# mbzuai-oryx/Video-LLaVA

Measured on NVIDIA H100. Metric: videos/sec (100-frame CLIP encode + 7B 32-tok decode), higher is better.
Workload: dtype bf16

## Files before the change

### video-llava_b200/csrc/attention_tc.cu

```cuda
#include "common.cuh"
#include "kernels.h"

#include <stdlib.h>

namespace vcl {

namespace {

constexpr int VA_WG = 2;
constexpr int VA_THREADS = VA_WG * 128;
constexpr int VA_TILE = 64 * 128;
constexpr int VA_KEY_TILES = 5;
constexpr int VA_OFF_K = 0;
constexpr int VA_OFF_VT = VA_OFF_K + VA_KEY_TILES * VA_TILE;
constexpr int VA_OFF_Q = VA_OFF_VT + VA_KEY_TILES * VA_TILE;
constexpr int VA_OFF_P = VA_OFF_Q + VA_WG * VA_TILE;
constexpr int VA_OFF_BAR = VA_OFF_P + VA_WG * VA_KEY_TILES * VA_TILE;
constexpr int VA_SMEM = VA_OFF_BAR + 64 + 1024;
static_assert(VA_SMEM <= 227 * 1024, "shared memory");

__device__ __forceinline__ uint32_t va_sw128(int row, int chunk) {
  return (uint32_t)row * 128u + (uint32_t)((chunk ^ (row & 7)) << 4);
}

__device__ __forceinline__ void named_bar_sync_wg(int id) { asm volatile("bar.sync %0, 128;" ::"r"(id) : "memory"); }

__global__ void __launch_bounds__(VA_THREADS, 1)
attn_vit_tc_kernel(const __grid_constant__ CUtensorMap tmap, const bf16* __restrict__ qkv, bf16* __restrict__ out,
                   int S, int H, int C) {
  extern __shared__ uint8_t smem_raw[];
  const uint32_t raw_addr = smem_u32(smem_raw);
  const uint32_t pad = ((raw_addr + 1023u) & ~1023u) - raw_addr;
  uint8_t* smem = smem_raw + pad;
  const uint32_t sbase = raw_addr + pad;
  const uint32_t kbar = sbase + VA_OFF_BAR;
  auto qbar = [&](int w) { return sbase + VA_OFF_BAR + 8u * (1 + w); };

  const int frame = blockIdx.x / H, h = blockIdx.x - frame * H;
  const int row0 = frame * S;
  const int wg = threadIdx.x >> 7, t = threadIdx.x & 127, lane = threadIdx.x & 31, wq = t >> 5;
  const int n_qt = (S + 63) / 64;
  const int n_kt = (S + 63) / 64;

  if (threadIdx.x == 0) {
    tma_prefetch_desc(&tmap);
    mbar_init(kbar, 1);
    for (int w = 0; w < VA_WG; ++w) mbar_init(qbar(w), 1);
    mbar_fence_init();
  }
  __syncthreads();
  if (threadIdx.x == 0) {
    mbar_arrive_expect_tx(kbar, n_kt * VA_TILE);
    for (int i = 0; i < n_kt; ++i) tma_load_2d(sbase + VA_OFF_K + i * VA_TILE, &tmap, kbar, C + h * 64, row0 + 64 * i);
    for (int w = 0; w < VA_WG && w < n_qt; ++w) {
      mbar_arrive_expect_tx(qbar(w), VA_TILE);
      tma_load_2d(sbase + VA_OFF_Q + w * VA_TILE, &tmap, qbar(w), h * 64, row0 + 64 * w);
    }
  }
  const bf16* vg = qkv + (long long)row0 * 3 * C + 2 * C + h * 64;
  for (int idx = threadIdx.x; idx < VA_KEY_TILES * 64 * 8; idx += VA_THREADS) {
    const int key = idx % (VA_KEY_TILES * 64), c = idx / (VA_KEY_TILES * 64);
    uint4 v = make_uint4(0u, 0u, 0u, 0u);
    if (key < S) v = *reinterpret_cast<const uint4*>(vg + (long long)key * 3 * C + c * 8);
    const uint32_t w4[4] = {v.x, v.y, v.z, v.w};
    uint8_t* tile = smem + VA_OFF_VT + (key >> 6) * VA_TILE;
    const int kc = (key & 63) >> 3, ke = key & 7;
#pragma unroll
    for (int e = 0; e < 8; ++e) {
      const uint16_t hv = (uint16_t)(e & 1 ? w4[e >> 1] >> 16 : w4[e >> 1] & 0xffffu);
      *reinterpret_cast<uint16_t*>(tile + va_sw128(c * 8 + e, kc) + ke * 2) = hv;
    }
  }
  asm volatile("fence.proxy.async.shared::cta;" ::: "memory");
  __syncthreads();
  mbar_wait(kbar, 0);

  const int r0 = 16 * wq + (lane >> 2), c2 = 2 * (lane & 3);
  const bool tail = S > 256;
  uint8_t* P = smem + VA_OFF_P + wg * VA_KEY_TILES * VA_TILE;
  const uint32_t p_addr = sbase + VA_OFF_P + wg * VA_KEY_TILES * VA_TILE;
  const uint32_t q_addr = sbase + VA_OFF_Q + wg * VA_TILE;
  uint32_t qphase = 0;
  float s[128], s2[16], o[32];
  for (int qt = wg; qt < n_qt; qt += VA_WG) {
    mbar_wait(qbar(wg), qphase);
    qphase ^= 1u;
#pragma unroll
    for (int i = 0; i < 128; ++i) s[i] = 0.f;
#pragma unroll
    for (int i = 0; i < 16; ++i) s2[i] = 0.f;
    wgmma_fence();
#pragma unroll
    for (int k = 0; k < 4; ++k) {
      const uint64_t ad = wgmma_desc_k_sw128(q_addr) + 2u * k;
      wgmma_bf16<256>(s, ad, wgmma_desc_k_sw128(sbase + VA_OFF_K) + 2u * k, k > 0 ? 1u : 0u);
      if (tail) wgmma_bf16<32>(s2, ad, wgmma_desc_k_sw128(sbase + VA_OFF_K + 256 * 128) + 2u * k, k > 0 ? 1u : 0u);
    }
    wgmma_commit();
    wgmma_wait<0>();
    wgmma_fence_regs(s);
    wgmma_fence_regs(s2);
    named_bar_sync_wg(1 + wg);
    if (t == 0 && qt + VA_WG < n_qt) {
      mbar_arrive_expect_tx(qbar(wg), VA_TILE);
      tma_load_2d(q_addr, &tmap, qbar(wg), h * 64, row0 + 64 * (qt + VA_WG));
    }
    auto sc = [&](float x, int key) { return key < S ? bf16r(bf16r(x) * 0.125f) : -INFINITY; };
    float m[2] = {-INFINITY, -INFINITY};
    uint32_t sp[64], sp2[8];
    auto pack_sc = [&](const float* a, int i, int key0) {
      const int hh = i & 1, col = key0 + 8 * (i >> 1) + c2;
      const float x0 = sc(a[2 * i], col), x1 = sc(a[2 * i + 1], col + 1);
      m[hh] = fmaxf(m[hh], fmaxf(x0, x1));
      return pack_bf16x2(x0, x1);
    };
    if (tail) {
#pragma unroll
      for (int i = 0; i < 8; ++i) sp2[i] = pack_sc(s2, i, 256);
    }
#pragma unroll
    for (int i = 0; i < 64; ++i) sp[i] = pack_sc(s, i, 0);
    float l[2] = {0.f, 0.f};
#pragma unroll
    for (int r = 0; r < 2; ++r) {
      m[r] = fmaxf(m[r], __shfl_xor_sync(0xffffffffu, m[r], 1));
      m[r] = fmaxf(m[r], __shfl_xor_sync(0xffffffffu, m[r], 2));
    }
    auto put_p = [&](uint32_t x2, int i, int key0) {
      const int hh = i & 1, row = r0 + 8 * hh, col = key0 + 8 * (i >> 1) + c2;
      const float p0 = exp2f((bf16lo(x2) - m[hh]) * 1.4426950408889634f);
      const float p1 = exp2f((bf16hi(x2) - m[hh]) * 1.4426950408889634f);
      l[hh] += p0 + p1;
      *reinterpret_cast<uint32_t*>(P + (col >> 6) * VA_TILE + va_sw128(row, (col & 63) >> 3) + (col & 7) * 2) =
          pack_bf16x2(p0, p1);
    };
#pragma unroll
    for (int i = 0; i < 64; ++i) put_p(sp[i], i, 0);
    if (tail) {
#pragma unroll
      for (int i = 0; i < 8; ++i) put_p(sp2[i], i, 256);
    }
    asm volatile("fence.proxy.async.shared::cta;" ::: "memory");
    named_bar_sync_wg(1 + wg);
#pragma unroll
    for (int i = 0; i < 32; ++i) o[i] = 0.f;
    wgmma_fence();
#pragma unroll
    for (int kk = 0; kk < 16; ++kk)
      wgmma_bf16<64>(o, wgmma_desc_k_sw128(p_addr + (kk >> 2) * VA_TILE) + 2u * (kk & 3),
                     wgmma_desc_k_sw128(sbase + VA_OFF_VT + (kk >> 2) * VA_TILE) + 2u * (kk & 3), kk > 0 ? 1u : 0u);
    if (tail)
      wgmma_bf16<64>(o, wgmma_desc_k_sw128(p_addr + 4 * VA_TILE), wgmma_desc_k_sw128(sbase + VA_OFF_VT + 4 * VA_TILE), 1u);
    wgmma_commit();
    wgmma_wait<0>();
    wgmma_fence_regs(o);
#pragma unroll
    for (int r = 0; r < 2; ++r) {
      l[r] += __shfl_xor_sync(0xffffffffu, l[r], 1);
      l[r] += __shfl_xor_sync(0xffffffffu, l[r], 2);
    }
#pragma unroll
    for (int hh = 0; hh < 2; ++hh) {
      const int q = qt * 64 + r0 + 8 * hh;
      if (q < S) {
        const float inv = 1.0f / l[hh];
        bf16* dst = out + (long long)(row0 + q) * C + h * 64 + c2;
#pragma unroll
        for (int j = 0; j < 8; ++j)
          *reinterpret_cast<uint32_t*>(dst + 8 * j) = pack_bf16x2(o[4 * j + 2 * hh] * inv, o[4 * j + 2 * hh + 1] * inv);
      }
    }
  }
}

}

int init_attention_tc_kernels() {
  VCL_CUDA_OK(cudaFuncSetAttribute(attn_vit_tc_kernel, cudaFuncAttributeMaxDynamicSharedMemorySize, VA_SMEM));
  return 0;
}

bool attention_vit_tc_supported(int S) {
  const bool off = getenv("VCL_VIT_ATTN_FLASH") != nullptr;
  return !off && S >= 129 && S <= 257;
}

int launch_attention_vit_tc(const bf16* qkv, bf16* out, int n_frames, int S, int H, int C, cudaStream_t stream) {
  VCL_REQUIRE(C == H * 64, "attention_vit_tc: head_dim must be 64");
  VCL_REQUIRE(S >= 129 && S <= 257, "attention_vit_tc: S=%d outside 129..257", S);
  VCL_REQUIRE(((uintptr_t)qkv % 16) == 0 && ((uintptr_t)out % 16) == 0, "attention_vit_tc: pointers must be 16-byte aligned");
  CUtensorMap tm;
  if (make_tmap_2d(&tm, qkv, (long long)n_frames * S, 3LL * C, 3LL * C, 64) != 0) return -2;
  attn_vit_tc_kernel<<<n_frames * H, VA_THREADS, VA_SMEM, stream>>>(tm, qkv, out, S, H, C);
  VCL_CUDA_OK(cudaGetLastError());
  count_launches(1);
  return 0;
}

}
```

### video-llava_b200/csrc/common.cuh

```cuda
#pragma once

#include <cuda.h>
#include <cuda_bf16.h>
#include <cuda_fp16.h>
#include <cuda_runtime.h>
#include <stdint.h>

namespace vcl {

typedef __nv_bfloat16 bf16;

void set_last_error(const char* fmt, ...);

#define VCL_CUDA_OK(expr)                                                                      \
  do {                                                                                         \
    cudaError_t _e = (expr);                                                                   \
    if (_e != cudaSuccess) {                                                                   \
      ::vcl::set_last_error("%s:%d: %s -> %s", __FILE__, __LINE__, #expr, cudaGetErrorString(_e)); \
      return -2;                                                                               \
    }                                                                                          \
  } while (0)

#define VCL_REQUIRE(cond, ...)                 \
  do {                                         \
    if (!(cond)) {                             \
      ::vcl::set_last_error(__VA_ARGS__);      \
      return -1;                               \
    }                                          \
  } while (0)

__device__ __forceinline__ float bf16r(float x) { return __bfloat162float(__float2bfloat16_rn(x)); }

__device__ __forceinline__ uint32_t pack_bf16x2(float lo, float hi) {
  __nv_bfloat162 v = __floats2bfloat162_rn(lo, hi);
  return *reinterpret_cast<uint32_t*>(&v);
}
__device__ __forceinline__ float bf16lo(uint32_t v) { return __uint_as_float(v << 16); }
__device__ __forceinline__ float bf16hi(uint32_t v) { return __uint_as_float(v & 0xffff0000u); }

__device__ __forceinline__ uint32_t bf16x2_mul(uint32_t a, uint32_t b) {
  __nv_bfloat162 r = __hmul2(*reinterpret_cast<__nv_bfloat162*>(&a), *reinterpret_cast<__nv_bfloat162*>(&b));
  return *reinterpret_cast<uint32_t*>(&r);
}
__device__ __forceinline__ uint32_t bf16x2_add(uint32_t a, uint32_t b) {
  __nv_bfloat162 r = __hadd2(*reinterpret_cast<__nv_bfloat162*>(&a), *reinterpret_cast<__nv_bfloat162*>(&b));
  return *reinterpret_cast<uint32_t*>(&r);
}

__device__ __forceinline__ float warp_sum(float v) {
#pragma unroll
  for (int o = 16; o > 0; o >>= 1) v += __shfl_xor_sync(0xffffffffu, v, o);
  return v;
}
__device__ __forceinline__ float warp_max(float v) {
#pragma unroll
  for (int o = 16; o > 0; o >>= 1) v = fmaxf(v, __shfl_xor_sync(0xffffffffu, v, o));
  return v;
}

__device__ __forceinline__ uint4 ld_nc_v4(const void* p) {
  uint4 r;
  asm volatile("ld.global.nc.L1::no_allocate.v4.u32 {%0,%1,%2,%3}, [%4];"
               : "=r"(r.x), "=r"(r.y), "=r"(r.z), "=r"(r.w)
               : "l"(p));
  return r;
}

__device__ __forceinline__ uint32_t smem_u32(const void* p) {
  return static_cast<uint32_t>(__cvta_generic_to_shared(p));
}

__device__ __forceinline__ void mbar_init(uint32_t bar, uint32_t count) {
  asm volatile("mbarrier.init.shared::cta.b64 [%0], %1;" ::"r"(bar), "r"(count) : "memory");
}
__device__ __forceinline__ void mbar_fence_init() {
  asm volatile("fence.mbarrier_init.release.cluster;" ::: "memory");
  asm volatile("fence.proxy.async.shared::cta;" ::: "memory");
}
__device__ __forceinline__ void mbar_arrive_expect_tx(uint32_t bar, uint32_t bytes) {
  asm volatile("mbarrier.arrive.expect_tx.shared::cta.b64 _, [%0], %1;" ::"r"(bar), "r"(bytes)
               : "memory");
}
__device__ __forceinline__ void mbar_arrive(uint32_t bar) {
  asm volatile("mbarrier.arrive.shared::cta.b64 _, [%0];" ::"r"(bar) : "memory");
}
__device__ __forceinline__ void mbar_wait(uint32_t bar, uint32_t parity) {
  asm volatile(
      "{\n\t"
      ".reg .pred p;\n\t"
      "VCL_WAIT_%=:\n\t"
      "mbarrier.try_wait.parity.shared::cta.b64 p, [%0], %1;\n\t"
      "@p bra VCL_DONE_%=;\n\t"
      "bra VCL_WAIT_%=;\n\t"
      "VCL_DONE_%=:\n\t"
      "}\n" ::"r"(bar),
      "r"(parity)
      : "memory");
}

__device__ __forceinline__ void tma_prefetch_desc(const void* tmap) {
  asm volatile("prefetch.tensormap [%0];" ::"l"(tmap) : "memory");
}
__device__ __forceinline__ void tma_load_2d(uint32_t dst_smem, const void* tmap, uint32_t bar,
                                            int32_t c0, int32_t c1) {
  asm volatile(
      "cp.async.bulk.tensor.2d.shared::cluster.global.mbarrier::complete_tx::bytes"
      " [%0], [%1, {%3, %4}], [%2];" ::"r"(dst_smem),
      "l"(tmap), "r"(bar), "r"(c0), "r"(c1)
      : "memory");
}

__device__ __forceinline__ void tma_prefetch_2d(const void* tmap, int32_t c0, int32_t c1) {
  asm volatile("cp.async.bulk.prefetch.tensor.2d.L2.global.tile [%0, {%1, %2}];" ::"l"(tmap), "r"(c0), "r"(c1)
               : "memory");
}

__device__ __forceinline__ void tma_load_2d_mc(uint32_t dst_smem, const void* tmap, uint32_t bar,
                                               int32_t c0, int32_t c1, uint16_t cta_mask) {
  asm volatile(
      "cp.async.bulk.tensor.2d.shared::cluster.global.mbarrier::complete_tx::bytes.multicast::cluster"
      " [%0], [%1, {%3, %4}], [%2], %5;" ::"r"(dst_smem),
      "l"(tmap), "r"(bar), "r"(c0), "r"(c1), "h"(cta_mask)
      : "memory");
}

__device__ __forceinline__ uint32_t cluster_ctarank() {
  uint32_t r;
  asm volatile("mov.u32 %0, %%cluster_ctarank;" : "=r"(r));
  return r;
}
__device__ __forceinline__ void cluster_sync_all() {
  asm volatile("barrier.cluster.arrive.release.aligned;" ::: "memory");
  asm volatile("barrier.cluster.wait.acquire.aligned;" ::: "memory");
}

__device__ __forceinline__ uint32_t mapa_cluster(uint32_t smem_addr, uint32_t cta_rank) {
  uint32_t r;
  asm volatile("mapa.shared::cluster.u32 %0, %1, %2;" : "=r"(r) : "r"(smem_addr), "r"(cta_rank));
  return r;
}
__device__ __forceinline__ void mbar_arrive_cluster(uint32_t bar_cluster_addr) {
  asm volatile("mbarrier.arrive.release.cluster.shared::cluster.b64 _, [%0];" ::"r"(bar_cluster_addr) : "memory");
}

__device__ __forceinline__ void wgmma_fence() { asm volatile("wgmma.fence.sync.aligned;" ::: "memory"); }
__device__ __forceinline__ void wgmma_commit() { asm volatile("wgmma.commit_group.sync.aligned;" ::: "memory"); }
template <int N>
__device__ __forceinline__ void wgmma_wait() {
  asm volatile("wgmma.wait_group.sync.aligned %0;" ::"n"(N) : "memory");
}
template <int R>
__device__ __forceinline__ void wgmma_fence_regs(float (&d)[R]) {
#pragma unroll
  for (int i = 0; i < R; ++i) asm volatile("" : "+f"(d[i])::"memory");
}
template <int R>
__device__ __forceinline__ void setmaxnreg_inc() { asm volatile("setmaxnreg.inc.sync.aligned.u32 %0;" ::"n"(R)); }
template <int R>
__device__ __forceinline__ void setmaxnreg_dec() { asm volatile("setmaxnreg.dec.sync.aligned.u32 %0;" ::"n"(R)); }

__device__ __forceinline__ uint64_t wgmma_desc_k_sw128(uint32_t smem_addr) {
  uint64_t d = 0;
  d |= (uint64_t)((smem_addr & 0x3ffffu) >> 4);
  d |= (uint64_t)1 << 16;
  d |= (uint64_t)(1024u >> 4) << 32;
  d |= (uint64_t)1 << 62;
  return d;
}

template <int N>
__device__ __forceinline__ void wgmma_bf16(float (&d)[N / 2], uint64_t adesc, uint64_t bdesc, uint32_t accumulate);
template <>
__device__ __forceinline__ void wgmma_bf16<256>(float (&d)[128], uint64_t adesc, uint64_t bdesc, uint32_t accumulate) {
  asm volatile(
      "{\n\t.reg .pred p;\n\tsetp.ne.b32 p, %130, 0;\n\t"
      "wgmma.mma_async.sync.aligned.m64n256k16.f32.bf16.bf16 {%0, %1, %2, %3, %4, %5, %6, %7, %8, %9, %10, %11, %12, %13, %14, %15, %16, %17, %18, %19, %20, %21, %22, %23, %24, %25, %26, %27, %28, %29, %30, %31, %32, %33, %34, %35, %36, %37, %38, %39, %40, %41, %42, %43, %44, %45, %46, %47, %48, %49, %50, %51, %52, %53, %54, %55, %56, %57, %58, %59, %60, %61, %62, %63, %64, %65, %66, %67, %68, %69, %70, %71, %72, %73, %74, %75, %76, %77, %78, %79, %80, %81, %82, %83, %84, %85, %86, %87, %88, %89, %90, %91, %92, %93, %94, %95, %96, %97, %98, %99, %100, %101, %102, %103, %104, %105, %106, %107, %108, %109, %110, %111, %112, %113, %114, %115, %116, %117, %118, %119, %120, %121, %122, %123, %124, %125, %126, %127}, %128, %129, p, 1, 1, 0, 0;\n\t}"
      : "+f"(d[0]), "+f"(d[1]), "+f"(d[2]), "+f"(d[3]), "+f"(d[4]), "+f"(d[5]), "+f"(d[6]), "+f"(d[7]), "+f"(d[8]), "+f"(d[9]), "+f"(d[10]), "+f"(d[11]), "+f"(d[12]), "+f"(d[13]), "+f"(d[14]), "+f"(d[15]), "+f"(d[16]), "+f"(d[17]), "+f"(d[18]), "+f"(d[19]), "+f"(d[20]), "+f"(d[21]), "+f"(d[22]), "+f"(d[23]), "+f"(d[24]), "+f"(d[25]), "+f"(d[26]), "+f"(d[27]), "+f"(d[28]), "+f"(d[29]), "+f"(d[30]), "+f"(d[31]), "+f"(d[32]), "+f"(d[33]), "+f"(d[34]), "+f"(d[35]), "+f"(d[36]), "+f"(d[37]), "+f"(d[38]), "+f"(d[39]), "+f"(d[40]), "+f"(d[41]), "+f"(d[42]), "+f"(d[43]), "+f"(d[44]), "+f"(d[45]), "+f"(d[46]), "+f"(d[47]), "+f"(d[48]), "+f"(d[49]), "+f"(d[50]), "+f"(d[51]), "+f"(d[52]), "+f"(d[53]), "+f"(d[54]), "+f"(d[55]), "+f"(d[56]), "+f"(d[57]), "+f"(d[58]), "+f"(d[59]), "+f"(d[60]), "+f"(d[61]), "+f"(d[62]), "+f"(d[63]), "+f"(d[64]), "+f"(d[65]), "+f"(d[66]), "+f"(d[67]), "+f"(d[68]), "+f"(d[69]), "+f"(d[70]), "+f"(d[71]), "+f"(d[72]), "+f"(d[73]), "+f"(d[74]), "+f"(d[75]), "+f"(d[76]), "+f"(d[77]), "+f"(d[78]), "+f"(d[79]), "+f"(d[80]), "+f"(d[81]), "+f"(d[82]), "+f"(d[83]), "+f"(d[84]), "+f"(d[85]), "+f"(d[86]), "+f"(d[87]), "+f"(d[88]), "+f"(d[89]), "+f"(d[90]), "+f"(d[91]), "+f"(d[92]), "+f"(d[93]), "+f"(d[94]), "+f"(d[95]), "+f"(d[96]), "+f"(d[97]), "+f"(d[98]), "+f"(d[99]), "+f"(d[100]), "+f"(d[101]), "+f"(d[102]), "+f"(d[103]), "+f"(d[104]), "+f"(d[105]), "+f"(d[106]), "+f"(d[107]), "+f"(d[108]), "+f"(d[109]), "+f"(d[110]), "+f"(d[111]), "+f"(d[112]), "+f"(d[113]), "+f"(d[114]), "+f"(d[115]), "+f"(d[116]), "+f"(d[117]), "+f"(d[118]), "+f"(d[119]), "+f"(d[120]), "+f"(d[121]), "+f"(d[122]), "+f"(d[123]), "+f"(d[124]), "+f"(d[125]), "+f"(d[126]), "+f"(d[127])
      : "l"(adesc), "l"(bdesc), "r"(accumulate));
}
template <>
__device__ __forceinline__ void wgmma_bf16<128>(float (&d)[64], uint64_t adesc, uint64_t bdesc, uint32_t accumulate) {
  asm volatile(
      "{\n\t.reg .pred p;\n\tsetp.ne.b32 p, %66, 0;\n\t"
      "wgmma.mma_async.sync.aligned.m64n128k16.f32.bf16.bf16 {%0, %1, %2, %3, %4, %5, %6, %7, %8, %9, %10, %11, %12, %13, %14, %15, %16, %17, %18, %19, %20, %21, %22, %23, %24, %25, %26, %27, %28, %29, %30, %31, %32, %33, %34, %35, %36, %37, %38, %39, %40, %41, %42, %43, %44, %45, %46, %47, %48, %49, %50, %51, %52, %53, %54, %55, %56, %57, %58, %59, %60, %61, %62, %63}, %64, %65, p, 1, 1, 0, 0;\n\t}"
      : "+f"(d[0]), "+f"(d[1]), "+f"(d[2]), "+f"(d[3]), "+f"(d[4]), "+f"(d[5]), "+f"(d[6]), "+f"(d[7]), "+f"(d[8]), "+f"(d[9]), "+f"(d[10]), "+f"(d[11]), "+f"(d[12]), "+f"(d[13]), "+f"(d[14]), "+f"(d[15]), "+f"(d[16]), "+f"(d[17]), "+f"(d[18]), "+f"(d[19]), "+f"(d[20]), "+f"(d[21]), "+f"(d[22]), "+f"(d[23]), "+f"(d[24]), "+f"(d[25]), "+f"(d[26]), "+f"(d[27]), "+f"(d[28]), "+f"(d[29]), "+f"(d[30]), "+f"(d[31]), "+f"(d[32]), "+f"(d[33]), "+f"(d[34]), "+f"(d[35]), "+f"(d[36]), "+f"(d[37]), "+f"(d[38]), "+f"(d[39]), "+f"(d[40]), "+f"(d[41]), "+f"(d[42]), "+f"(d[43]), "+f"(d[44]), "+f"(d[45]), "+f"(d[46]), "+f"(d[47]), "+f"(d[48]), "+f"(d[49]), "+f"(d[50]), "+f"(d[51]), "+f"(d[52]), "+f"(d[53]), "+f"(d[54]), "+f"(d[55]), "+f"(d[56]), "+f"(d[57]), "+f"(d[58]), "+f"(d[59]), "+f"(d[60]), "+f"(d[61]), "+f"(d[62]), "+f"(d[63])
      : "l"(adesc), "l"(bdesc), "r"(accumulate));
}
template <>
__device__ __forceinline__ void wgmma_bf16<64>(float (&d)[32], uint64_t adesc, uint64_t bdesc, uint32_t accumulate) {
  asm volatile(
      "{\n\t.reg .pred p;\n\tsetp.ne.b32 p, %34, 0;\n\t"
      "wgmma.mma_async.sync.aligned.m64n64k16.f32.bf16.bf16 {%0, %1, %2, %3, %4, %5, %6, %7, %8, %9, %10, %11, %12, %13, %14, %15, %16, %17, %18, %19, %20, %21, %22, %23, %24, %25, %26, %27, %28, %29, %30, %31}, %32, %33, p, 1, 1, 0, 0;\n\t}"
      : "+f"(d[0]), "+f"(d[1]), "+f"(d[2]), "+f"(d[3]), "+f"(d[4]), "+f"(d[5]), "+f"(d[6]), "+f"(d[7]), "+f"(d[8]), "+f"(d[9]), "+f"(d[10]), "+f"(d[11]), "+f"(d[12]), "+f"(d[13]), "+f"(d[14]), "+f"(d[15]), "+f"(d[16]), "+f"(d[17]), "+f"(d[18]), "+f"(d[19]), "+f"(d[20]), "+f"(d[21]), "+f"(d[22]), "+f"(d[23]), "+f"(d[24]), "+f"(d[25]), "+f"(d[26]), "+f"(d[27]), "+f"(d[28]), "+f"(d[29]), "+f"(d[30]), "+f"(d[31])
      : "l"(adesc), "l"(bdesc), "r"(accumulate));
}
template <>
__device__ __forceinline__ void wgmma_bf16<32>(float (&d)[16], uint64_t adesc, uint64_t bdesc, uint32_t accumulate) {
  asm volatile(
      "{\n\t.reg .pred p;\n\tsetp.ne.b32 p, %18, 0;\n\t"
      "wgmma.mma_async.sync.aligned.m64n32k16.f32.bf16.bf16 {%0, %1, %2, %3, %4, %5, %6, %7, %8, %9, %10, %11, %12, %13, %14, %15}, %16, %17, p, 1, 1, 0, 0;\n\t}"
      : "+f"(d[0]), "+f"(d[1]), "+f"(d[2]), "+f"(d[3]), "+f"(d[4]), "+f"(d[5]), "+f"(d[6]), "+f"(d[7]), "+f"(d[8]), "+f"(d[9]), "+f"(d[10]), "+f"(d[11]), "+f"(d[12]), "+f"(d[13]), "+f"(d[14]), "+f"(d[15])
      : "l"(adesc), "l"(bdesc), "r"(accumulate));
}

}
```

### video-llava_b200/csrc/gemm_tc.cu

```cuda
#include "common.cuh"
#include "kernels.h"

#include <cudaTypedefs.h>

namespace vcl {

template <int BLOCK_N>
struct GemmCfg {
  static constexpr int BLOCK_M = 128;
  static constexpr int BLOCK_K = 64;
  static constexpr int A_BYTES = BLOCK_M * BLOCK_K * 2;
  static constexpr int B_BYTES = BLOCK_N * BLOCK_K * 2;
  static constexpr int STAGE_BYTES = A_BYTES + B_BYTES;
  static constexpr int OUT_PITCH = BLOCK_N * 2 + 16;
  static constexpr int OUT_BYTES = BLOCK_M * OUT_PITCH;
  static constexpr int BAR_BYTES = 256;
  static constexpr int STAGES = (BLOCK_N == 256) ? 3 : (BLOCK_N == 128 ? 5 : 8);
  static constexpr int SMEM_BYTES = STAGES * STAGE_BYTES + BAR_BYTES + OUT_BYTES + 1024;
  static_assert((2 * STAGES + 4) * 8 <= BAR_BYTES, "barrier area");
  static_assert(SMEM_BYTES <= 227 * 1024, "shared memory");
};

__device__ __forceinline__ float act_gelu_erf(float x) {
  x = bf16r(x);
// ... 256 lines not shown
          wgmma_bf16<BLOCK_N>(acc, a_desc + 2u * k, b_desc + 2u * k, (kb | k) != 0 ? 1u : 0u);
        }
        wgmma_commit();
        wgmma_wait<1>();
        if (prev >= 0) release(prev);
        prev = stage;
        if (++stage == STAGES) { stage = 0; phase ^= 1u; }
      }
      wgmma_wait<0>();
      release(prev);
      wgmma_fence_regs(acc);
      if (tile != cluster_id) {
        mbar_wait(drained_bar(cw), out_phase);
        out_phase ^= 1u;
      }
      gemm_epilogue_stage<BLOCK_N, ACT>(acc, stg, lane, wq, m_blk * Cfg::BLOCK_M + cw * 64, n_blk, bias, M, N, rope);
      mbar_arrive(staged_bar(cw));
    }
  }

  __syncthreads();
  if (CL > 1) cluster_sync_all();
}

static PFN_cuTensorMapEncodeTiled_v12000 g_encode = nullptr;
static int resolve_encode() {
  if (g_encode) return 0;
  void* fn = nullptr;
  cudaDriverEntryPointQueryResult qres;
  cudaError_t e = cudaGetDriverEntryPoint("cuTensorMapEncodeTiled", &fn, cudaEnableDefault, &qres);
  if (e != cudaSuccess || fn == nullptr || qres != cudaDriverEntryPointSuccess) {
    set_last_error("cuTensorMapEncodeTiled is not available from the driver (%s)",
                   cudaGetErrorString(e));
    return -2;
  }
  g_encode = reinterpret_cast<PFN_cuTensorMapEncodeTiled_v12000>(fn);
  return 0;
}

int make_tmap_2d(CUtensorMap* out, const void* ptr, long long rows, long long cols, long long ld,
                 int box_rows) {
  if (resolve_encode() != 0) return -2;
  cuuint64_t gdim[2] = {(cuuint64_t)cols, (cuuint64_t)rows};
  cuuint64_t gstride[1] = {(cuuint64_t)ld * 2};
  cuuint32_t box[2] = {64u, (cuuint32_t)box_rows};
  cuuint32_t estr[2] = {1u, 1u};
  CUresult r = g_encode(out, CU_TENSOR_MAP_DATA_TYPE_BFLOAT16, 2, const_cast<void*>(ptr), gdim,
                        gstride, box, estr, CU_TENSOR_MAP_INTERLEAVE_NONE,
                        CU_TENSOR_MAP_SWIZZLE_128B, CU_TENSOR_MAP_L2_PROMOTION_L2_256B,
                        CU_TENSOR_MAP_FLOAT_OOB_FILL_NONE);
  if (r != CUDA_SUCCESS) {
    set_last_error("cuTensorMapEncodeTiled failed (%d) ptr=%p rows=%lld cols=%lld ld=%lld box=%d",
                   (int)r, ptr, rows, cols, ld, box_rows);
    return -2;
  }
  return 0;
}

static int g_num_sms = 0;
int device_num_sms() {
  if (g_num_sms == 0) {
    int dev = 0;
    cudaGetDevice(&dev);
    cudaDeviceGetAttribute(&g_num_sms, cudaDevAttrMultiProcessorCount, dev);
    if (g_num_sms <= 0) g_num_sms = 132;
  }
  return g_num_sms;
}

template <int BLOCK_N, int ACT, int CL>
static int launch_one(const GemmArgs& g, cudaStream_t stream) {
  using Cfg = GemmCfg<BLOCK_N>;
  auto kern = gemm_bf16_tn_kernel<BLOCK_N, ACT, CL>;
  CUtensorMap ta, tb;
  if (make_tmap_2d(&ta, g.A, g.M, g.K, g.lda, Cfg::BLOCK_M) != 0) return -2;
  if (make_tmap_2d(&tb, g.W, g.N, g.K, g.ldw, BLOCK_N / CL) != 0) return -2;
  const int num_m = (g.M + 127) / 128;
  const int num_tiles = ((num_m + CL - 1) / CL) * ((g.N + BLOCK_N - 1) / BLOCK_N);
  cudaLaunchConfig_t cfg = {};
  cfg.blockDim = dim3(384);
  cfg.dynamicSmemBytes = Cfg::SMEM_BYTES;
  cfg.stream = stream;
  cudaLaunchAttribute attr[1];
  attr[0].id = cudaLaunchAttributeClusterDimension;
  attr[0].val.clusterDim.x = CL;
  attr[0].val.clusterDim.y = 1;
  attr[0].val.clusterDim.z = 1;
  cfg.attrs = attr;
  cfg.numAttrs = CL > 1 ? 1 : 0;
  static int resident = 0;
  if (resident == 0) {
    if (CL > 1) {
      cfg.gridDim = dim3(CL);
      VCL_CUDA_OK(cudaOccupancyMaxActiveClusters(&resident, kern, &cfg));
    }
    if (resident <= 0) resident = device_num_sms() / CL;
  }
  int clusters = resident;
  if (clusters > num_tiles) clusters = num_tiles;
  if (g.max_ctas > 0 && clusters * CL > g.max_ctas) clusters = g.max_ctas / CL > 0 ? g.max_ctas / CL : 1;
  cfg.gridDim = dim3(clusters * CL);
  VCL_CUDA_OK(cudaLaunchKernelEx(&cfg, kern, ta, tb, g.C, (long long)g.ldc, g.bias, g.residual,
                                 (long long)g.ldr, g.M, g.N, g.K, g.rope));
  count_launches(1);
  return 0;
}
// ... 107 lines not shown
```

### video-llava_b200/csrc/kernels.h

```cpp
#pragma once

#include <cuda.h>
#include <cuda_bf16.h>
#include <cuda_runtime.h>
#include <stdint.h>

namespace vcl {

typedef __nv_bfloat16 bf16;

constexpr int PACK_SEQ_MAX = 64;
constexpr int PACK_HEAD = 6 * PACK_SEQ_MAX;
inline size_t pack_elems(long long rows) { return PACK_HEAD + 2 * (size_t)rows; }
template <class T> __host__ __device__ inline T* pack_off(T* p) { return p; }
template <class T> __host__ __device__ inline T* pack_len(T* p) { return p + PACK_SEQ_MAX; }
template <class T> __host__ __device__ inline T* pack_slot(T* p) { return p + 2 * PACK_SEQ_MAX; }
template <class T> __host__ __device__ inline T* pack_last(T* p) { return p + 3 * PACK_SEQ_MAX; }
template <class T> __host__ __device__ inline T* pack_start(T* p) { return p + 4 * PACK_SEQ_MAX; }
template <class T> __host__ __device__ inline T* pack_end(T* p) { return p + 5 * PACK_SEQ_MAX; }
template <class T> __host__ __device__ inline T* pack_row(T* p, long long r) { return p + PACK_HEAD + 2 * r; }

struct KvPages {
  const int* table = nullptr;
  int row = 0;
  long long blk = 0;
};
__device__ __forceinline__ long long kv_paged_off(const KvPages& p, int slot, int head, int col) {
  return (long long)__ldg(p.table + slot * p.row + (col >> 7)) * p.blk + ((long long)head * 128 + (col & 127)) * 128;
}

enum Act { ACT_NONE = 0, ACT_QGELU = 1, ACT_GELU = 2, ACT_SWIGLU = 3, ACT_ROPE = 4 };
struct RopeEpilogue {
  const bf16* cos_t = nullptr; const bf16* sin_t = nullptr;
  bf16* kcache = nullptr; bf16* vcache = nullptr;
  int S = 0, start_pos = 0, H = 0, s_max = 0;
  const int* n_pad = nullptr;
  const int* pack = nullptr;
  KvPages pages;
};


void set_last_error(const char* fmt, ...);
void count_launches(long long n);
long long launch_count();
int device_num_sms();

struct GemmArgs {
  const bf16* A = nullptr;  long long lda = 0;
  const bf16* W = nullptr;  long long ldw = 0;
  bf16* C = nullptr;        long long ldc = 0;
  const bf16* bias = nullptr;
  const bf16* residual = nullptr; long long ldr = 0;
  int M = 0, N = 0, K = 0;
  int act = ACT_NONE;
  int block_n = 0;
  int cluster = 0;
  int max_ctas = 0;
  RopeEpilogue rope;
};
int launch_gemm_bf16_tn(const GemmArgs& g, cudaStream_t stream);
int init_gemm_kernels();
int make_tmap_2d(CUtensorMap* out, const void* ptr, long long rows, long long cols, long long ld,
                 int box_rows);

int launch_layernorm(const bf16* x, long long ldx, bf16* y, long long ldy, const bf16* w,
                     const bf16* b, int rows, int D, float eps, cudaStream_t stream);
int launch_rmsnorm(const bf16* x, long long ldx, bf16* y, long long ldy, const bf16* w, int rows,
                   int D, float eps, cudaStream_t stream);
int launch_im2col(const void* pixels, int mode, bf16* out, int n_frames, int image, int patch,
                  int KP, cudaStream_t stream);
int launch_clip_embed_ln(const bf16* patch_out, const bf16* cls, const bf16* pos, const bf16* ln_w,
                         const bf16* ln_b, bf16* h, int n_frames, int P, int D, float eps,
                         cudaStream_t stream);
int launch_embed_splice(const long long* ids, const bf16* table, const bf16* vid, const int* vid_start,
                        bf16* h, int B, int S, int D, int n_vid, int vocab, cudaStream_t stream,
                        const int* pack = nullptr, int M = 0);
int launch_rope_table(bf16* cos_t, bf16* sin_t, int max_pos, int head_dim, float theta,
                      cudaStream_t stream);
int launch_rope_kv_prefill(bf16* qkv, bf16* kcache, bf16* vcache, const bf16* cos_t,
                           const bf16* sin_t, int B, int S, int H, int head_dim, int s_max, int pos0,
                           cudaStream_t stream, const int* pos_dev = nullptr, const int* n_pad = nullptr);
int launch_embed_tokens(const int* tok, long long tok_stride, const bf16* table, bf16* h, int B,
                        int D, int vocab, cudaStream_t stream);
int launch_argmax(const float* logits, int* out, long long out_stride, int B, int V,
                  cudaStream_t stream);
int launch_fill_int(int* dst, int value, int n, cudaStream_t stream);

int launch_st_pool(const void* feats, int in_dtype, long long frame_stride, long long patch_stride,
                   int T, int P, int C, int n_temporal, void* out, int out_dtype,
                   cudaStream_t stream);

int launch_cross_entropy(const bf16* logits, long long ld, int V, const long long* labels, long long row0, int rows,
                         int seg, float* nll, bf16* logits_out, cudaStream_t stream);
int launch_nll_mean(const float* nll, const long long* labels, long long rows, int seg, float* nll_out,
                    float* loss_out, cudaStream_t stream);

#ifndef VCL_LOGPROBS_MAX
#define VCL_LOGPROBS_MAX 20
#endif
#ifndef VCL_SAMPLE_WIDE_MAX_V
#define VCL_SAMPLE_WIDE_MAX_V 57344
#endif
struct SampleArgs {
  const float* logits = nullptr; long long ld = 0; int V = 0, B = 0;
  const float* temperature = nullptr; const int* top_k = nullptr; const unsigned long long* seed = nullptr;
  int entry0 = 0; const int* rowmap = nullptr;
  int col = 0; const int* col_dev = nullptr; const int* n_pad = nullptr;
  int* out = nullptr; long long out_stride = 1;
  const int* top_n = nullptr;
  int* lp_id = nullptr; float* lp_val = nullptr;
  long long lp_entry = 0, lp_pos = 0; int lp_rows = 0;
  const float* top_p = nullptr; const float* rep = nullptr;
  unsigned int* tset = nullptr; int tset_words = 0;
};
int launch_sample(const SampleArgs& a, cudaStream_t stream);
// ... 104 lines not shown
```

Measured before the change: 5.147.

## Make ViT attention persistent and warp-specialized with TMA producer and register-sourced PV

Rewrites the CLIP ViT attention kernel as a persistent kernel with a dedicated producer warpgroup that TMA-loads K, V and Q tiles into double-buffered stages guarded by mbarriers, while two consumer warpgroups compute. V is now loaded by TMA and consumed via an MN-major descriptor instead of a manual transpose into shared memory. P stays in registers and feeds a register-sourced wgmma, avoiding the shared-memory P round trip. It also splits the QK wgmma in two to overlap softmax with the second half and does the scale and max in packed bf16x2. This adds register-reallocation and barrier complexity, and the bf16 rounding of the scaled score differs slightly from before.

```diff
diff --git a/video-llava_b200/csrc/attention_tc.cu b/video-llava_b200/csrc/attention_tc.cu
--- a/video-llava_b200/csrc/attention_tc.cu
+++ b/video-llava_b200/csrc/attention_tc.cu
@@ -7,176 +7,210 @@
 
 namespace {
 
-constexpr int VA_WG = 2;
-constexpr int VA_THREADS = VA_WG * 128;
+constexpr int VA_CWG = 2;
+constexpr int VA_THREADS = (1 + VA_CWG) * 128;
 constexpr int VA_TILE = 64 * 128;
 constexpr int VA_KEY_TILES = 5;
-constexpr int VA_OFF_K = 0;
-constexpr int VA_OFF_VT = VA_OFF_K + VA_KEY_TILES * VA_TILE;
-constexpr int VA_OFF_Q = VA_OFF_VT + VA_KEY_TILES * VA_TILE;
-constexpr int VA_OFF_P = VA_OFF_Q + VA_WG * VA_TILE;
-constexpr int VA_OFF_BAR = VA_OFF_P + VA_WG * VA_KEY_TILES * VA_TILE;
-constexpr int VA_SMEM = VA_OFF_BAR + 64 + 1024;
+constexpr int VA_STAGES = 2;
+constexpr int VA_QSLOTS = 6;
+constexpr int VA_STAGE = 2 * VA_KEY_TILES * VA_TILE;
+constexpr int VA_OFF_Q = VA_STAGES * VA_STAGE;
+constexpr int VA_OFF_BAR = VA_OFF_Q + VA_QSLOTS * VA_TILE;
+constexpr int VA_SMEM = VA_OFF_BAR + 8 * (2 * VA_STAGES + 2 * VA_QSLOTS) + 1024;
 static_assert(VA_SMEM <= 227 * 1024, "shared memory");
 
-__device__ __forceinline__ uint32_t va_sw128(int row, int chunk) {
-  return (uint32_t)row * 128u + (uint32_t)((chunk ^ (row & 7)) << 4);
-}
-
-__device__ __forceinline__ void named_bar_sync_wg(int id) { asm volatile("bar.sync %0, 128;" ::"r"(id) : "memory"); }
-
+template <bool TAIL>
 __global__ void __launch_bounds__(VA_THREADS, 1)
-attn_vit_tc_kernel(const __grid_constant__ CUtensorMap tmap, const bf16* __restrict__ qkv, bf16* __restrict__ out,
-                   int S, int H, int C) {
+attn_vit_tc_kernel(const __grid_constant__ CUtensorMap tmap, bf16* __restrict__ out, int n_frames, int S, int H,
+                   int C) {
   extern __shared__ uint8_t smem_raw[];
   const uint32_t raw_addr = smem_u32(smem_raw);
-  const uint32_t pad = ((raw_addr + 1023u) & ~1023u) - raw_addr;
-  uint8_t* smem = smem_raw + pad;
-  const uint32_t sbase = raw_addr + pad;
-  const uint32_t kbar = sbase + VA_OFF_BAR;
-  auto qbar = [&](int w) { return sbase + VA_OFF_BAR + 8u * (1 + w); };
-
-  const int frame = blockIdx.x / H, h = blockIdx.x - frame * H;
-  const int row0 = frame * S;
-  const int wg = threadIdx.x >> 7, t = threadIdx.x & 127, lane = threadIdx.x & 31, wq = t >> 5;
+  const uint32_t sbase = (raw_addr + 1023u) & ~1023u;
+  const uint32_t bars = sbase + VA_OFF_BAR;
+  auto kv_full = [&](int s) { return bars + 8u * s; };
+  auto kv_empty = [&](int s) { return bars + 8u * (VA_STAGES + s); };
+  auto q_full = [&](int i) { return bars + 8u * (2 * VA_STAGES + i); };
+  auto q_empty = [&](int i) { return bars + 8u * (2 * VA_STAGES + VA_QSLOTS + i); };
+
+  const int n_items = n_frames * H;
   const int n_qt = (S + 63) / 64;
-  const int n_kt = (S + 63) / 64;
+  constexpr int N_KT = TAIL ? 5 : 4;
+  const int wg = threadIdx.x >> 7;
 
   if (threadIdx.x == 0) {
     tma_prefetch_desc(&tmap);
-    mbar_init(kbar, 1);
-    for (int w = 0; w < VA_WG; ++w) mbar_init(qbar(w), 1);
+    for (int s = 0; s < VA_STAGES; ++s) {
+      mbar_init(kv_full(s), 1);
+      mbar_init(kv_empty(s), 4 * VA_CWG);
+    }
+    for (int i = 0; i < VA_QSLOTS; ++i) {
+      mbar_init(q_full(i), 1);
+      mbar_init(q_empty(i), 4);
+    }
     mbar_fence_init();
   }
   __syncthreads();
-  if (threadIdx.x == 0) {
-    mbar_arrive_expect_tx(kbar, n_kt * VA_TILE);
-    for (int i = 0; i < n_kt; ++i) tma_load_2d(sbase + VA_OFF_K + i * VA_TILE, &tmap, kbar, C + h * 64, row0 + 64 * i);
-    for (int w = 0; w < VA_WG && w < n_qt; ++w) {
-      mbar_arrive_expect_tx(qbar(w), VA_TILE);
-      tma_load_2d(sbase + VA_OFF_Q + w * VA_TILE, &tmap, qbar(w), h * 64, row0 + 64 * w);
-    }
+
+  if (wg == 0) {
+    setmaxnreg_dec<40>();
+    if (threadIdx.x == 0) {
+      int g = 0;
+      for (int it = blockIdx.x, j = 0; it < n_items; it += gridDim.x, ++j) {
+        const int frame = it / H, h = it - frame * H;
+        const int st = j % VA_STAGES;
+        mbar_wait(kv_empty(st), ((j / VA_STAGES) & 1) ^ 1u);
+        mbar_arrive_expect_tx(kv_full(st), 2 * N_KT * VA_TILE);
+        const uint32_t k_dst = sbase + st * VA_STAGE;
+        for (int i = 0; i < N_KT; ++i) {
+          tma_load_3d(k_dst + i * VA_TILE, &tmap, kv_full(st), C + h * 64, 64 * i, frame);
+          tma_load_3d(k_dst + (VA_KEY_TILES + i) * VA_TILE, &tmap, kv_full(st), 2 * C + h * 64, 64 * i, frame);
+        }
+        for (int qt = 0; qt < n_qt; ++qt, ++g) {
+          const int slot = g % VA_QSLOTS;
+          mbar_wait(q_empty(slot), ((g / VA_QSLOTS) & 1) ^ 1u);
+          mbar_arrive_expect_tx(q_full(slot), VA_TILE);
+          tma_load_3d(sbase + VA_OFF_Q + slot * VA_TILE, &tmap, q_full(slot), h * 64, 64 * qt, frame);
+        }
+      }
+    }
+    return;
   }
-  const bf16* vg = qkv + (long long)row0 * 3 * C + 2 * C + h * 64;
-  for (int idx = threadIdx.x; idx < VA_KEY_TILES * 64 * 8; idx += VA_THREADS) {
-    const int key = idx % (VA_KEY_TILES * 64), c = idx / (VA_KEY_TILES * 64);
-    uint4 v = make_uint4(0u, 0u, 0u, 0u);
-    if (key < S) v = *reinterpret_cast<const uint4*>(vg + (long long)key * 3 * C + c * 8);
-    const uint32_t w4[4] = {v.x, v.y, v.z, v.w};
-    uint8_t* tile = smem + VA_OFF_VT + (key >> 6) * VA_TILE;
-    const int kc = (key & 63) >> 3, ke = key & 7;
-#pragma unroll
-    for (int e = 0; e < 8; ++e) {
-      const uint16_t hv = (uint16_t)(e & 1 ? w4[e >> 1] >> 16 : w4[e >> 1] & 0xffffu);
-      *reinterpret_cast<uint16_t*>(tile + va_sw128(c * 8 + e, kc) + ke * 2) = hv;
+
+  setmaxnreg_inc<232>();
+  const int cw = wg - 1, t = threadIdx.x & 127, lane = threadIdx.x & 31, wq = t >> 5;
+  const int r0 = 16 * wq + (lane >> 2), c2 = 2 * (lane & 3);
+  float s[128], s2[16], o[32];
+  int g0 = 0;
+  for (int it = blockIdx.x, j = 0; it < n_items; it += gridDim.x, ++j, g0 += n_qt) {
+    const int frame = it / H, h = it - frame * H;
+    const int st = j % VA_STAGES;
+    const uint32_t k_addr = sbase + st * VA_STAGE, v_addr = k_addr + VA_KEY_TILES * VA_TILE;
+    mbar_wait(kv_full(st), (j / VA_STAGES) & 1);
+    for (int qt = (cw ^ g0) & 1; qt < n_qt; qt += 2) {
+      const int slot = (g0 + qt) % VA_QSLOTS;
+      const uint32_t q_addr = sbase + VA_OFF_Q + slot * VA_TILE;
+      mbar_wait(q_full(slot), ((g0 + qt) / VA_QSLOTS) & 1);
+#pragma unroll
+      for (int i = 0; i < 128; ++i) s[i] = 0.f;
+#pragma unroll
+      for (int i = 0; i < 16; ++i) s2[i] = 0.f;
+      float(&s_lo)[64] = *reinterpret_cast<float(*)[64]>(s);
+      float(&s_hi)[64] = *reinterpret_cast<float(*)[64]>(s + 64);
+      wgmma_fence();
+#pragma unroll
+      for (int k = 0; k < 4; ++k)
+        wgmma_bf16<128>(s_lo, wgmma_desc_k_sw128(q_addr) + 2u * k, wgmma_desc_k_sw128(k_addr) + 2u * k, k > 0 ? 1u : 0u);
+      wgmma_commit();
+#pragma unroll
+      for (int k = 0; k < 4; ++k) {
+        const uint64_t ad = wgmma_desc_k_sw128(q_addr) + 2u * k;
+        wgmma_bf16<128>(s_hi, ad, wgmma_desc_k_sw128(k_addr + 128 * 128) + 2u * k, k > 0 ? 1u : 0u);
+        if constexpr (TAIL) wgmma_bf16<32>(s2, ad, wgmma_desc_k_sw128(k_addr + 256 * 128) + 2u * k, k > 0 ? 1u : 0u);
+      }
+      wgmma_commit();
+      uint32_t p[64], p2[4];
+      float l[2] = {0.f, 0.f};
+      if (qt * 64 + 16 * wq < S) {
+        uint32_t mx[2] = {0xff80ff80u, 0xff80ff80u};
+        auto score = [&](const float* a, int i, int key0, bool may_mask) {
+          const int col = key0 + 8 * (i >> 1) + c2;
+          uint32_t v = bf16x2_mul(pack_bf16x2(a[2 * i], a[2 * i + 1]), 0x3e003e00u);
+          if (may_mask) {
+            if (col >= S) v = (v & 0xffff0000u) | 0xff80u;
+            if (col + 1 >= S) v = (v & 0xffffu) | 0xff800000u;
+          }
+          mx[i & 1] = bf16x2_max(mx[i & 1], v);
+          return v;
+        };
+        wgmma_wait<1>();
+        wgmma_fence_regs(s_lo);
+#pragma unroll
+        for (int i = 0; i < 32; ++i) p[i] = score(s, i, 0, false);
+        wgmma_wait<0>();
+        wgmma_fence_regs(s_hi);
+        wgmma_fence_regs(s2);
+        __syncwarp();
+        if (lane == 0) mbar_arrive(q_empty(slot));
+        if constexpr (TAIL) {
+#pragma unroll
+          for (int i = 0; i < 4; ++i) p2[i] = score(s2, i, 256, true);
+        }
+#pragma unroll
+        for (int i = 32; i < 64; ++i) p[i] = score(s, i, 0, !TAIL);
+        float m[2] = {fmaxf(bf16lo(mx[0]), bf16hi(mx[0])), fmaxf(bf16lo(mx[1]), bf16hi(mx[1]))};
+#pragma unroll
+        for (int r = 0; r < 2; ++r) {
+          m[r] = fmaxf(m[r], __shfl_xor_sync(0xffffffffu, m[r], 1));
+          m[r] = fmaxf(m[r], __shfl_xor_sync(0xffffffffu, m[r], 2));
+        }
+        auto exp_p = [&](uint32_t x2, int i) {
+          const int hh = i & 1;
+          const float p0 = exp2f((bf16lo(x2) - m[hh]) * 1.4426950408889634f);
+          const float p1 = exp2f((bf16hi(x2) - m[hh]) * 1.4426950408889634f);
+          l[hh] += p0 + p1;
+          return pack_bf16x2(p0, p1);
+        };
+#pragma unroll
+        for (int i = 0; i < 64; ++i) p[i] = exp_p(p[i], i);
+        if constexpr (TAIL) {
+#pragma unroll
+          for (int i = 0; i < 4; ++i) p2[i] = exp_p(p2[i], i);
+        }
+      } else {
+        wgmma_wait<0>();
+        wgmma_fence_regs(s);
+        wgmma_fence_regs(s2);
+        __syncwarp();
+        if (lane == 0) mbar_arrive(q_empty(slot));
+#pragma unroll
+        for (int i = 0; i < 64; ++i) p[i] = 0u;
+#pragma unroll
+        for (int i = 0; i < 4; ++i) p2[i] = 0u;
+      }
+#pragma unroll
+      for (int i = 0; i < 32; ++i) o[i] = 0.f;
+      wgmma_fence();
+#pragma unroll
+      for (int kk = 0; kk < 16; ++kk)
+        wgmma_bf16_rs_n64_bmn(o, p[4 * kk], p[4 * kk + 1], p[4 * kk + 2], p[4 * kk + 3],
+                              wgmma_desc_mn_sw128(v_addr + (kk >> 2) * VA_TILE + (kk & 3) * 2048), kk > 0 ? 1u : 0u);
+      if constexpr (TAIL) wgmma_bf16_rs_n64_bmn(o, p2[0], p2[1], p2[2], p2[3], wgmma_desc_mn_sw128(v_addr + 4 * VA_TILE), 1u);
+      wgmma_commit();
+      wgmma_wait<0>();
+      wgmma_fence_regs(o);
+#pragma unroll
+      for (int i = 0; i < 64; ++i) asm volatile("" : "+r"(p[i])::"memory");
+#pragma unroll
+      for (int i = 0; i < 4; ++i) asm volatile("" : "+r"(p2[i])::"memory");
+      if (qt + 2 >= n_qt) {
+        __syncwarp();
+        if (lane == 0) mbar_arrive(kv_empty(st));
+      }
+#pragma unroll
+      for (int r = 0; r < 2; ++r) {
+        l[r] += __shfl_xor_sync(0xffffffffu, l[r], 1);
+        l[r] += __shfl_xor_sync(0xffffffffu, l[r], 2);
+      }
+#pragma unroll
+      for (int hh = 0; hh < 2; ++hh) {
+        const int q = qt * 64 + r0 + 8 * hh;
+        if (q < S) {
+          const float inv = 1.0f / l[hh];
+          bf16* dst = out + ((long long)frame * S + q) * C + h * 64 + c2;
+#pragma unroll
+          for (int jj = 0; jj < 8; ++jj)
+            *reinterpret_cast<uint32_t*>(dst + 8 * jj) = pack_bf16x2(o[4 * jj + 2 * hh] * inv, o[4 * jj + 2 * hh + 1] * inv);
+        }
+      }
     }
   }
-  asm volatile("fence.proxy.async.shared::cta;" ::: "memory");
-  __syncthreads();
-  mbar_wait(kbar, 0);
-
-  const int r0 = 16 * wq + (lane >> 2), c2 = 2 * (lane & 3);
-  const bool tail = S > 256;
-  uint8_t* P = smem + VA_OFF_P + wg * VA_KEY_TILES * VA_TILE;
-  const uint32_t p_addr = sbase + VA_OFF_P + wg * VA_KEY_TILES * VA_TILE;
-  const uint32_t q_addr = sbase + VA_OFF_Q + wg * VA_TILE;
-  uint32_t qphase = 0;
-  float s[128], s2[16], o[32];
-  for (int qt = wg; qt < n_qt; qt += VA_WG) {
-    mbar_wait(qbar(wg), qphase);
-    qphase ^= 1u;
-#pragma unroll
-    for (int i = 0; i < 128; ++i) s[i] = 0.f;
-#pragma unroll
-    for (int i = 0; i < 16; ++i) s2[i] = 0.f;
-    wgmma_fence();
-#pragma unroll
-    for (int k = 0; k < 4; ++k) {
-      const uint64_t ad = wgmma_desc_k_sw128(q_addr) + 2u * k;
-      wgmma_bf16<256>(s, ad, wgmma_desc_k_sw128(sbase + VA_OFF_K) + 2u * k, k > 0 ? 1u : 0u);
-      if (tail) wgmma_bf16<32>(s2, ad, wgmma_desc_k_sw128(sbase + VA_OFF_K + 256 * 128) + 2u * k, k > 0 ? 1u : 0u);
-    }
-    wgmma_commit();
-    wgmma_wait<0>();
-    wgmma_fence_regs(s);
-    wgmma_fence_regs(s2);
-    named_bar_sync_wg(1 + wg);
-    if (t == 0 && qt + VA_WG < n_qt) {
-      mbar_arrive_expect_tx(qbar(wg), VA_TILE);
-      tma_load_2d(q_addr, &tmap, qbar(wg), h * 64, row0 + 64 * (qt + VA_WG));
-    }
-    auto sc = [&](float x, int key) { return key < S ? bf16r(bf16r(x) * 0.125f) : -INFINITY; };
-    float m[2] = {-INFINITY, -INFINITY};
-    uint32_t sp[64], sp2[8];
-    auto pack_sc = [&](const float* a, int i, int key0) {
-      const int hh = i & 1, col = key0 + 8 * (i >> 1) + c2;
-      const float x0 = sc(a[2 * i], col), x1 = sc(a[2 * i + 1], col + 1);
-      m[hh] = fmaxf(m[hh], fmaxf(x0, x1));
-      return pack_bf16x2(x0, x1);
-    };
-    if (tail) {
-#pragma unroll
-      for (int i = 0; i < 8; ++i) sp2[i] = pack_sc(s2, i, 256);
-    }
-#pragma unroll
-    for (int i = 0; i < 64; ++i) sp[i] = pack_sc(s, i, 0);
-    float l[2] = {0.f, 0.f};
-#pragma unroll
-    for (int r = 0; r < 2; ++r) {
-      m[r] = fmaxf(m[r], __shfl_xor_sync(0xffffffffu, m[r], 1));
-      m[r] = fmaxf(m[r], __shfl_xor_sync(0xffffffffu, m[r], 2));
-    }
-    auto put_p = [&](uint32_t x2, int i, int key0) {
-      const int hh = i & 1, row = r0 + 8 * hh, col = key0 + 8 * (i >> 1) + c2;
-      const float p0 = exp2f((bf16lo(x2) - m[hh]) * 1.4426950408889634f);
-      const float p1 = exp2f((bf16hi(x2) - m[hh]) * 1.4426950408889634f);
-      l[hh] += p0 + p1;
-      *reinterpret_cast<uint32_t*>(P + (col >> 6) * VA_TILE + va_sw128(row, (col & 63) >> 3) + (col & 7) * 2) =
-          pack_bf16x2(p0, p1);
-    };
-#pragma unroll
-    for (int i = 0; i < 64; ++i) put_p(sp[i], i, 0);
-    if (tail) {
-#pragma unroll
-      for (int i = 0; i < 8; ++i) put_p(sp2[i], i, 256);
-    }
-    asm volatile("fence.proxy.async.shared::cta;" ::: "memory");
-    named_bar_sync_wg(1 + wg);
-#pragma unroll
-    for (int i = 0; i < 32; ++i) o[i] = 0.f;
-    wgmma_fence();
-#pragma unroll
-    for (int kk = 0; kk < 16; ++kk)
-      wgmma_bf16<64>(o, wgmma_desc_k_sw128(p_addr + (kk >> 2) * VA_TILE) + 2u * (kk & 3),
-                     wgmma_desc_k_sw128(sbase + VA_OFF_VT + (kk >> 2) * VA_TILE) + 2u * (kk & 3), kk > 0 ? 1u : 0u);
-    if (tail)
-      wgmma_bf16<64>(o, wgmma_desc_k_sw128(p_addr + 4 * VA_TILE), wgmma_desc_k_sw128(sbase + VA_OFF_VT + 4 * VA_TILE), 1u);
-    wgmma_commit();
-    wgmma_wait<0>();
-    wgmma_fence_regs(o);
-#pragma unroll
-    for (int r = 0; r < 2; ++r) {
-      l[r] += __shfl_xor_sync(0xffffffffu, l[r], 1);
-      l[r] += __shfl_xor_sync(0xffffffffu, l[r], 2);
-    }
-#pragma unroll
-    for (int hh = 0; hh < 2; ++hh) {
-      const int q = qt * 64 + r0 + 8 * hh;
-      if (q < S) {
-        const float inv = 1.0f / l[hh];
-        bf16* dst = out + (long long)(row0 + q) * C + h * 64 + c2;
-#pragma unroll
-        for (int j = 0; j < 8; ++j)
-          *reinterpret_cast<uint32_t*>(dst + 8 * j) = pack_bf16x2(o[4 * j + 2 * hh] * inv, o[4 * j + 2 * hh + 1] * inv);
-      }
-    }
-  }
 }
 
 }
 
 int init_attention_tc_kernels() {
-  VCL_CUDA_OK(cudaFuncSetAttribute(attn_vit_tc_kernel, cudaFuncAttributeMaxDynamicSharedMemorySize, VA_SMEM));
+  VCL_CUDA_OK(cudaFuncSetAttribute(attn_vit_tc_kernel<false>, cudaFuncAttributeMaxDynamicSharedMemorySize, VA_SMEM));
+  VCL_CUDA_OK(cudaFuncSetAttribute(attn_vit_tc_kernel<true>, cudaFuncAttributeMaxDynamicSharedMemorySize, VA_SMEM));
   return 0;
 }
 
@@ -190,8 +224,10 @@
   VCL_REQUIRE(S >= 129 && S <= 257, "attention_vit_tc: S=%d outside 129..257", S);
   VCL_REQUIRE(((uintptr_t)qkv % 16) == 0 && ((uintptr_t)out % 16) == 0, "attention_vit_tc: pointers must be 16-byte aligned");
   CUtensorMap tm;
-  if (make_tmap_2d(&tm, qkv, (long long)n_frames * S, 3LL * C, 3LL * C, 64) != 0) return -2;
-  attn_vit_tc_kernel<<<n_frames * H, VA_THREADS, VA_SMEM, stream>>>(tm, qkv, out, S, H, C);
+  if (make_tmap_3d(&tm, qkv, n_frames, S, 3LL * C, 3LL * C, 64) != 0) return -2;
+  const int items = n_frames * H, sms = device_num_sms();
+  auto kern = S > 256 ? attn_vit_tc_kernel<true> : attn_vit_tc_kernel<false>;
+  kern<<<items < sms ? items : sms, VA_THREADS, VA_SMEM, stream>>>(tm, out, n_frames, S, H, C);
   VCL_CUDA_OK(cudaGetLastError());
   count_launches(1);
   return 0;
diff --git a/video-llava_b200/csrc/common.cuh b/video-llava_b200/csrc/common.cuh
--- a/video-llava_b200/csrc/common.cuh
+++ b/video-llava_b200/csrc/common.cuh
@@ -44,6 +44,11 @@
 }
 __device__ __forceinline__ uint32_t bf16x2_add(uint32_t a, uint32_t b) {
   __nv_bfloat162 r = __hadd2(*reinterpret_cast<__nv_bfloat162*>(&a), *reinterpret_cast<__nv_bfloat162*>(&b));
+  return *reinterpret_cast<uint32_t*>(&r);
+}
+
+__device__ __forceinline__ uint32_t bf16x2_max(uint32_t a, uint32_t b) {
+  __nv_bfloat162 r = __hmax2(*reinterpret_cast<__nv_bfloat162*>(&a), *reinterpret_cast<__nv_bfloat162*>(&b));
   return *reinterpret_cast<uint32_t*>(&r);
 }
 
@@ -110,6 +115,15 @@
       : "memory");
 }
 
+__device__ __forceinline__ void tma_load_3d(uint32_t dst_smem, const void* tmap, uint32_t bar,
+                                            int32_t c0, int32_t c1, int32_t c2) {
+  asm volatile(
+      "cp.async.bulk.tensor.3d.shared::cluster.global.mbarrier::complete_tx::bytes"
+      " [%0], [%1, {%3, %4, %5}], [%2];" ::"r"(dst_smem),
+      "l"(tmap), "r"(bar), "r"(c0), "r"(c1), "r"(c2)
+      : "memory");
+}
+
 __device__ __forceinline__ void tma_prefetch_2d(const void* tmap, int32_t c0, int32_t c1) {
   asm volatile("cp.async.bulk.prefetch.tensor.2d.L2.global.tile [%0, {%1, %2}];" ::"l"(tmap), "r"(c0), "r"(c1)
                : "memory");
@@ -168,6 +182,15 @@
   return d;
 }
 
+__device__ __forceinline__ uint64_t wgmma_desc_mn_sw128(uint32_t smem_addr) {
+  uint64_t d = 0;
+  d |= (uint64_t)((smem_addr & 0x3ffffu) >> 4);
+  d |= (uint64_t)(8192u >> 4) << 16;
+  d |= (uint64_t)(1024u >> 4) << 32;
+  d |= (uint64_t)1 << 62;
+  return d;
+}
+
 template <int N>
 __device__ __forceinline__ void wgmma_bf16(float (&d)[N / 2], uint64_t adesc, uint64_t bdesc, uint32_t accumulate);
 template <>
@@ -203,4 +226,13 @@
       : "l"(adesc), "l"(bdesc), "r"(accumulate));
 }
 
-}
+__device__ __forceinline__ void wgmma_bf16_rs_n64_bmn(float (&d)[32], uint32_t a0, uint32_t a1, uint32_t a2,
+                                                      uint32_t a3, uint64_t bdesc, uint32_t accumulate) {
+  asm volatile(
+      "{\n\t.reg .pred p;\n\tsetp.ne.b32 p, %37, 0;\n\t"
+      "wgmma.mma_async.sync.aligned.m64n64k16.f32.bf16.bf16 {%0, %1, %2, %3, %4, %5, %6, %7, %8, %9, %10, %11, %12, %13, %14, %15, %16, %17, %18, %19, %20, %21, %22, %23, %24, %25, %26, %27, %28, %29, %30, %31}, {%32, %33, %34, %35}, %36, p, 1, 1, 1;\n\t}"
+      : "+f"(d[0]), "+f"(d[1]), "+f"(d[2]), "+f"(d[3]), "+f"(d[4]), "+f"(d[5]), "+f"(d[6]), "+f"(d[7]), "+f"(d[8]), "+f"(d[9]), "+f"(d[10]), "+f"(d[11]), "+f"(d[12]), "+f"(d[13]), "+f"(d[14]), "+f"(d[15]), "+f"(d[16]), "+f"(d[17]), "+f"(d[18]), "+f"(d[19]), "+f"(d[20]), "+f"(d[21]), "+f"(d[22]), "+f"(d[23]), "+f"(d[24]), "+f"(d[25]), "+f"(d[26]), "+f"(d[27]), "+f"(d[28]), "+f"(d[29]), "+f"(d[30]), "+f"(d[31])
+      : "r"(a0), "r"(a1), "r"(a2), "r"(a3), "l"(bdesc), "r"(accumulate));
+}
+
+}
diff --git a/video-llava_b200/csrc/gemm_tc.cu b/video-llava_b200/csrc/gemm_tc.cu
--- a/video-llava_b200/csrc/gemm_tc.cu
+++ b/video-llava_b200/csrc/gemm_tc.cu
@@ -332,6 +332,25 @@
   if (r != CUDA_SUCCESS) {
     set_last_error("cuTensorMapEncodeTiled failed (%d) ptr=%p rows=%lld cols=%lld ld=%lld box=%d",
                    (int)r, ptr, rows, cols, ld, box_rows);
+    return -2;
+  }
+  return 0;
+}
+
+int make_tmap_3d(CUtensorMap* out, const void* ptr, long long n, long long rows, long long cols, long long ld,
+                 int box_rows) {
+  if (resolve_encode() != 0) return -2;
+  cuuint64_t gdim[3] = {(cuuint64_t)cols, (cuuint64_t)rows, (cuuint64_t)n};
+  cuuint64_t gstride[2] = {(cuuint64_t)ld * 2, (cuuint64_t)(rows * ld * 2)};
+  cuuint32_t box[3] = {64u, (cuuint32_t)box_rows, 1u};
+  cuuint32_t estr[3] = {1u, 1u, 1u};
+  CUresult r = g_encode(out, CU_TENSOR_MAP_DATA_TYPE_BFLOAT16, 3, const_cast<void*>(ptr), gdim,
+                        gstride, box, estr, CU_TENSOR_MAP_INTERLEAVE_NONE,
+                        CU_TENSOR_MAP_SWIZZLE_128B, CU_TENSOR_MAP_L2_PROMOTION_L2_256B,
+                        CU_TENSOR_MAP_FLOAT_OOB_FILL_NONE);
+  if (r != CUDA_SUCCESS) {
+    set_last_error("cuTensorMapEncodeTiled failed (%d) ptr=%p n=%lld rows=%lld cols=%lld ld=%lld box=%d",
+                   (int)r, ptr, n, rows, cols, ld, box_rows);
     return -2;
   }
   return 0;
diff --git a/video-llava_b200/csrc/kernels.h b/video-llava_b200/csrc/kernels.h
--- a/video-llava_b200/csrc/kernels.h
+++ b/video-llava_b200/csrc/kernels.h
@@ -61,6 +61,8 @@
 int launch_gemm_bf16_tn(const GemmArgs& g, cudaStream_t stream);
 int init_gemm_kernels();
 int make_tmap_2d(CUtensorMap* out, const void* ptr, long long rows, long long cols, long long ld,
+                 int box_rows);
+int make_tmap_3d(CUtensorMap* out, const void* ptr, long long n, long long rows, long long cols, long long ld,
                  int box_rows);
 
 int launch_layernorm(const bf16* x, long long ldx, bf16* y, long long ldy, const bf16* w,
```

Measured after the change: 5.247, median of 6. 2.0% higher.
